# SciML/NonlinearSolve.jl

Hardware: NVIDIA H100
Metric: gmres_jvps_per_s (higher is better)
Workload: dtype f64

## Files before the change

nonlinearsolve.jl_b200/csrc/common.cuh:

```cuda
#pragma once
#include <cuda_runtime.h>
#include <stdint.h>
#include <stdio.h>
#include <string>
#include <vector>
#include "../../include/b200newton.h"

struct b200_ctx {
  int device = 0;
  cudaStream_t stream = nullptr;
  bool own_stream = false;
  int sm_count = 132;
  size_t smem_optin = 0;
  size_t l2_bytes = 0;
  std::string last_error;
  int64_t launches = 0;
  double* d_partials = nullptr;
  double* d_scalars = nullptr;
  double* h_scalars = nullptr;
  void* l2_flush = nullptr;
  size_t l2_flush_bytes = 0;
  cudaStream_t aux_stream = nullptr;
  cudaEvent_t ev_a = nullptr, ev_b = nullptr;
  unsigned long long* d_lu_xchg = nullptr;
  bool prof_on = false;
  struct ProfSlot { double ms = 0, bytes = 0; int64_t launches = 0; } prof[B200_KID_COUNT];
  struct ProfPending { int kid; double bytes; cudaEvent_t a, b; };
  std::vector<ProfPending> prof_pending;
  std::vector<cudaEvent_t> prof_free;
  void prof_begin(int kid, double bytes);
  void prof_end();
  void prof_collect();
  int32_t fail(int32_t code, const char* what, const char* file, int line);
};

#define PLAUNCH(ctx, kid, bytes, kernel, grid, block, smem, ...)                        \
  do {                                                                                  \
    if ((ctx)->prof_on) (ctx)->prof_begin((kid), (bytes));                              \
    kernel<<<(grid), (block), (smem), (ctx)->stream>>>(__VA_ARGS__);                    \
    (ctx)->launches++;                                                                  \
    if ((ctx)->prof_on) (ctx)->prof_end();                                              \
  } while (0)

#define B200_DEVICE_GUARD(ctxexpr)                                                      \
  do {                                                                                  \
    const b200_ctx* g__ = (ctxexpr);                                                    \
    int d__ = -1;                                                                       \
    if (g__ && (cudaGetDevice(&d__) != cudaSuccess || d__ != g__->device)) cudaSetDevice(g__->device); \
  } while (0)

#define B200_RED_MAX_BLOCKS 2048
enum { RED_DOT = 0, RED_SUMSQ = 1, RED_MAXABS = 2, RED_DIFFSQ = 3, RED_MIN = 4, RED_MAX = 5, RED_NEQ = 6,
       RED_SUMSQ2 = 7 , RED_MAXABS2 = 8 , RED_RELVIOL = 9 ,
       RED_COUNT_LE = 10 , RED_COUNT_DIFF_LE = 11  };

#define CUDA_TRY(ctx, expr)                                                             \
  do {                                                                                  \
    cudaError_t e__ = (expr);                                                           \
    if (e__ != cudaSuccess) {                                                           \
      char buf__[512];                                                                  \
      snprintf(buf__, sizeof(buf__), "%s -> %s", #expr, cudaGetErrorString(e__));       \
      return (ctx)->fail(B200_ERR_CUDA, buf__, __FILE__, __LINE__);                     \
    }                                                                                   \
  } while (0)

#define B200_TRY(expr)                  \
  do {                                  \
    int32_t s__ = (expr);               \
    if (s__ != B200_OK) return s__;     \
  } while (0)

#define B200_REQUIRE(ctx, cond, msg)                                                    \
  do {                                                                                  \
    if (!(cond)) return (ctx)->fail(B200_ERR_INVALID, msg, __FILE__, __LINE__);         \
  } while (0)

#define LAUNCH(ctx, kernel, grid, block, smem, ...)                                     \
  do {                                                                                  \
    kernel<<<(grid), (block), (smem), (ctx)->stream>>>(__VA_ARGS__);                    \
    (ctx)->launches++;                                                                  \
  } while (0)

#define CHECK_LAUNCH(ctx) CUDA_TRY(ctx, cudaPeekAtLastError())

__device__ __forceinline__ double warp_sum(double v) {
#pragma unroll
  for (int o = 16; o > 0; o >>= 1) v += __shfl_xor_sync(0xffffffffu, v, o);
  return v;
}
__device__ __forceinline__ double warp_max(double v) {
#pragma unroll
  for (int o = 16; o > 0; o >>= 1) v = fmax(v, __shfl_xor_sync(0xffffffffu, v, o));
  return v;
}
__device__ __forceinline__ double warp_min(double v) {
#pragma unroll
  for (int o = 16; o > 0; o >>= 1) v = fmin(v, __shfl_xor_sync(0xffffffffu, v, o));
  return v;
}
__device__ __forceinline__ double block_sum(double v, double* red) {
  const int lane = threadIdx.x & 31, wid = threadIdx.x >> 5, nw = (blockDim.x + 31) >> 5;
  v = warp_sum(v);
  __syncthreads();
  if (lane == 0) red[wid] = v;
  __syncthreads();
  v = (threadIdx.x < nw) ? red[threadIdx.x] : 0.0;
  if (wid == 0) v = warp_sum(v);
  return v;
}
__device__ __forceinline__ double block_max(double v, double* red) {
  const int lane = threadIdx.x & 31, wid = threadIdx.x >> 5, nw = (blockDim.x + 31) >> 5;
  v = warp_max(v);
  __syncthreads();
  if (lane == 0) red[wid] = v;
  __syncthreads();
  v = (threadIdx.x < nw) ? red[threadIdx.x] : 0.0;
  if (wid == 0) v = warp_max(v);
  return v;
}
__device__ __forceinline__ double abs_nf(double x) {
  double a = fabs(x);
  return (a == a) ? a : __longlong_as_double(0x7ff0000000000000LL);
}
__device__ __forceinline__ void atomic_max_nonneg(double* addr, double v) {
  atomicMax(reinterpret_cast<unsigned long long*>(addr), static_cast<unsigned long long>(__double_as_longlong(v)));
}

struct b200_problem {
  b200_ctx* ctx;
  int32_t kind;
  int32_t N;
  int64_t n;
  double A, B, alpha, a;
  double p;
  const double* pvec;
  b200_residual_cb f_cb;
  b200_jvp_cb jvp_cb, vjp_cb;
  b200_jac_cb jac_dense_cb, jac_nzval_cb;
  void* user;
  double* fd_scratch;
  int64_t *proto_colptr, *proto_rowval;
};

struct b200_sparse_jac;
struct b200_mg;

__device__ __forceinline__ void mbar_init(uint64_t* bar, unsigned count) {
  asm volatile("mbarrier.init.shared::cta.b64 [%0], %1;" ::"r"((unsigned)__cvta_generic_to_shared(bar)), "r"(count));
}
__device__ __forceinline__ void mbar_arrive(uint64_t* bar) {
  asm volatile("mbarrier.arrive.shared::cta.b64 _, [%0];" ::"r"((unsigned)__cvta_generic_to_shared(bar)) : "memory");
}
__device__ __forceinline__ void mbar_expect_tx(uint64_t* bar, unsigned bytes) {
  asm volatile("mbarrier.arrive.expect_tx.shared::cta.b64 _, [%0], %1;" ::"r"((unsigned)__cvta_generic_to_shared(bar)), "r"(bytes) : "memory");
}
__device__ __forceinline__ void mbar_wait(uint64_t* bar, unsigned parity) {
  const unsigned a = (unsigned)__cvta_generic_to_shared(bar);
  unsigned done = 0, spins = 0;
  while (!done) {
    asm volatile("{ .reg .pred p; mbarrier.try_wait.parity.shared::cta.b64 p, [%1], %2; selp.u32 %0, 1, 0, p; }" : "=r"(done) : "r"(a), "r"(parity) : "memory");
    if (++spins > (1u << 26)) break;
  }
}
__device__ __forceinline__ void tma_bulk_load(void* smem_dst, const void* gsrc, unsigned bytes, uint64_t* bar) {
  asm volatile("cp.async.bulk.shared::cluster.global.mbarrier::complete_tx::bytes [%0], [%1], %2, [%3];" ::"r"((unsigned)__cvta_generic_to_shared(smem_dst)),
               "l"(gsrc), "r"(bytes), "r"((unsigned)__cvta_generic_to_shared(bar))
               : "memory");
}
__device__ __forceinline__ void l2_bulk_prefetch(const void* gsrc, unsigned bytes) {
  asm volatile("cp.async.bulk.prefetch.L2.global [%0], %1;" ::"l"(gsrc), "r"(bytes) : "memory");
}

__device__ __forceinline__ void ll_store(unsigned long long* dst, unsigned long long v, unsigned epoch) {
  const unsigned long long e = (unsigned long long)epoch << 32;
  asm volatile("st.relaxed.gpu.global.v2.u64 [%0], {%1, %2};" ::"l"(dst), "l"((v & 0xffffffffull) | e), "l"((v >> 32) | e) : "memory");
}
__device__ __forceinline__ ulonglong2 ll_load(const unsigned long long* src) {
  ulonglong2 p;
  asm volatile("ld.relaxed.gpu.global.v2.u64 {%0, %1}, [%2];" : "=l"(p.x), "=l"(p.y) : "l"(src) : "memory");
  return p;
}
__device__ __forceinline__ void ll_wait(const unsigned long long* src, ulonglong2& p, unsigned epoch, unsigned bound, int* fault) {
  unsigned spins = 0;
  while ((unsigned)(p.x >> 32) != epoch || (unsigned)(p.y >> 32) != epoch) {
    if (++spins > bound) { *fault = 1; break; }
    p = ll_load(src);
  }
}
__device__ __forceinline__ unsigned long long ll_value(ulonglong2 p) { return (p.x & 0xffffffffull) | (p.y << 32); }


constexpr int32_t B200I_ENS_RC_DEFERRED = -7;

struct b200_linop {
  b200_ctx* ctx;
  int32_t kind;
  int64_t n;
  b200_problem* prob;
  const double* u;
  int32_t jvp_mode;
  const int64_t *colptr, *rowval;
  const double* nzval;
  int32_t index_base;
  const double* A;
  int64_t ld;
  b200_matvec_cb mv;
  void* user;
  b200_sparse_jac* sj;
  double shift;
  b200_mg* mg;
  int32_t owns_mg;
  int64_t *csr_rowptr, *csr_col, *csr_map;
  b200_ilu0* ilu;
};
enum { LINOP_PROBLEM = 0, LINOP_CSC = 1, LINOP_DENSE = 2, LINOP_CALLBACK = 3, LINOP_SPARSE_JAC = 4, LINOP_BLOCK_JACOBI = 5, LINOP_MULTIGRID = 6,
       LINOP_ILU0 = 7 };

static inline int32_t b200i_sync_for_callback(b200_ctx* ctx) {
  if (cudaStreamSynchronize(ctx->stream) != cudaSuccess) return B200_ERR_CUDA;
  if (ctx->aux_stream && cudaStreamSynchronize(ctx->aux_stream) != cudaSuccess) return B200_ERR_CUDA;
  return B200_OK;
}
int32_t b200i_linop_apply(b200_linop* op, const double* x, double* y);
int32_t b200i_mg_create(b200_problem* prob, b200_mg** out);
int32_t b200i_mg_destroy(b200_mg* mg);
int32_t b200i_mg_setup(b200_mg* mg, const double* u);
int32_t b200i_mg_apply(b200_mg* mg, const double* x, double* y);
int32_t b200i_mg_levels(b200_mg* mg, int32_t* nlev, int32_t* sizes, int32_t cap);
int32_t b200i_diag_shift(b200_ctx* ctx, int64_t n, double* A, int64_t ld, double shift);
int32_t b200i_qrcp_solve(b200_ctx* ctx, int64_t n, double* A, int64_t ld, double* b, double* x, double* work, int32_t* jpvt_dev, int32_t* rank_host);
int32_t b200i_gram(b200_ctx* ctx, int64_t n, const double* J, int64_t ld, double* C, int64_t ldc);
int32_t b200i_klement_descent(b200_ctx* ctx, int64_t n, const double* J, const double* fu, double* du);
int32_t b200i_klement_update(b200_ctx* ctx, int64_t n, double* J, const double* fu, double* fu_cache, const double* du);
int32_t b200i_ger(b200_ctx* ctx, int64_t n, double* A, int64_t ld, const double* c, const double* w);
int32_t b200i_scaled_identity(b200_ctx* ctx, int64_t n, double* A, int64_t ld, double d);
int32_t b200i_lm_damp(b200_ctx* ctx, int64_t n, double* C, int64_t ldc, double* dtd, double lambda);
void b200i_sparse_jac_csr(b200_sparse_jac* sj, const int64_t** rowptr, const int64_t** csr_col, const int64_t** csr_map);
int32_t b200i_residual_norm(b200_problem* prob, const double* u, double* du, double* d_norminf );
int32_t b200i_axpy_norm(b200_ctx* ctx, int64_t n, double a, const double* x, double* y, double* d_sumsq );
int32_t b200i_reduce_sum_dev(b200_ctx* ctx, int64_t n, const double* x, const double* y, int mode, double* d_out, double a = 0.0);
int32_t b200i_fetch_scalars(b200_ctx* ctx, int count);
```

nonlinearsolve.jl_b200/csrc/gmres.cu:

```cuda
#include "common.cuh"
#include <math.h>
#include <float.h>
#include <stdlib.h>
#include <algorithm>

namespace {
constexpr int GM_THREADS = 256;
constexpr int JT = 8;
constexpr int GM_KCAP = 16384;

struct GmresState {
  int32_t status;
  int32_t k;
  int32_t iter_base;
  int32_t itmax;
  int32_t kmax_cycle;
  int32_t pad;
  double rnorm0, rnorm, tol, atol, rtol, inv_h, hbis;
};

__device__ __forceinline__ void sym_givens(double a, double b, double& c, double& s, double& rho) {
  if (b == 0.0) {
    c = (a == 0.0) ? 1.0 : (a > 0 ? 1.0 : -1.0);
    s = 0.0;
// ... 368 lines not shown
    partial[(int64_t)threadIdx.x * G + blockIdx.x] = s;
  }
}
__global__ void tall_gemvt_final_kernel(int nc, int G, const double* __restrict__ partial, double* __restrict__ y) {
  const int c = threadIdx.x;
  if (c >= nc) return;
  double s = 0.0;
  for (int g = 0; g < G; ++g) s += partial[(int64_t)c * G + g];
  y[c] = s;
}
struct ResidentParams {
  int dim, N, k, passes, G;
  int opkind;
  const int64_t *rowptr, *csr_col, *csr_map;
  const double* nzval;
  int64_t NC;
  int cpc;
  int qs;
  double a, A;
  const double* u;
  const double* const* V;
  double* vnew;
  unsigned long long* slots;
  unsigned epoch_base;
  int* err;
  double* h;
  double* gsub;
  double *R, *cs, *sn, *z, *hraw;
  GmresState* st;
};

constexpr int LL_MAXG = 160;
constexpr int R3_POLLERS = LL_MAXG;
constexpr int R3_SPARE_POLLER = R3_POLLERS - 1;
constexpr int R3_THREADS = 256;
__device__ __forceinline__ void resident_givens_tail(const ResidentParams& P, double hbis, double inv, double* ws, int cap, int tid) {
  const int k = P.k;
  GmresState* st = P.st;
  double* Rk = P.R + (int64_t)(k - 1) * k / 2;
  double* hr = P.hraw ? P.hraw + (int64_t)(k - 1) * (k + 2) / 2 : nullptr;
  const bool staged = 3 * k <= cap;
  double *col, *cs, *sn;
  if (staged) {
    col = ws; cs = ws + k; sn = ws + 2 * k;
    for (int i = tid; i < k; i += R3_THREADS) {
      const double h = P.h[i];
      col[i] = h; cs[i] = P.cs[i]; sn[i] = P.sn[i];
      if (hr) hr[i] = h;
    }
    __syncthreads();
  } else {
    col = Rk; cs = P.cs; sn = P.sn;
    if (tid == 0) {
      for (int i = 0; i < k; ++i) { const double h = P.h[i]; Rk[i] = h; if (hr) hr[i] = h; }
    }
  }
  if (tid == 0) {
    if (hr) hr[k] = hbis;
    double x = col[0];
    for (int i = 0; i + 1 < k; ++i) {
      const double nx = col[i + 1];
      col[i] = cs[i] * x + sn[i] * nx;
      x = sn[i] * x - cs[i] * nx;
    }
    double c, s_, rho;
    sym_givens(x, hbis, c, s_, rho);
    P.cs[k - 1] = c; P.sn[k - 1] = s_; col[k - 1] = rho;
    const double zeta = s_ * P.z[k - 1];
    P.z[k - 1] = c * P.z[k - 1];
    P.z[k] = zeta;
    const double rnorm = fabs(zeta);
    st->rnorm = rnorm; st->hbis = hbis; st->k = k; st->inv_h = inv;
    st->status = *P.err ? B200_LS_NONFINITE : gm_step_status(rnorm, hbis, k, st);
  }
  if (staged) {
    __syncthreads();
    for (int i = tid; i < k; i += R3_THREADS) Rk[i] = col[i];
  }
}

constexpr int R3_RP = 30;
constexpr int R3_ROWS = 2 * R3_RP;
constexpr int R3_RPR = 16;
constexpr int R3_VR = 2 * R3_RPR;
constexpr size_t R3_ANNEX_BYTES = (size_t)(R3_RP - R3_RPR) * R3_THREADS * 16;
constexpr int R3_REPL = 16;
constexpr size_t R3_BUF_WORDS = (size_t)R3_REPL * LL_MAXG * 4;

constexpr unsigned R3_SPIN_BOUND = 1u << 22;

__device__ __forceinline__ void r3_post(unsigned long long* buf, int b, double a, double c, unsigned epoch) {
  const int lane = threadIdx.x;
  if (lane < R3_REPL) {
    unsigned long long* dst = buf + ((size_t)lane * LL_MAXG + b) * 4;
    ll_store(dst, (unsigned long long)__double_as_longlong(a), epoch);
    ll_store(dst + 2, (unsigned long long)__double_as_longlong(c), epoch);
  }
}
__device__ __forceinline__ void r3_poll(const unsigned long long* buf, int b, int G, unsigned epoch, int* err, double* gA, double* gC) {
  const int tid = threadIdx.x;
  if (tid < R3_POLLERS) {
    double xa = 0.0, xc = 0.0;
    if (tid < G) {
      const unsigned long long* src = buf + ((size_t)(b & (R3_REPL - 1)) * LL_MAXG + tid) * 4;
      unsigned long long a0, a1, c0, c1;
      unsigned spins = 0;
      bool ok;
      do {
        asm volatile("ld.relaxed.gpu.global.v2.u64 {%0, %1}, [%2];" : "=l"(a0), "=l"(a1) : "l"(src) : "memory");
        asm volatile("ld.relaxed.gpu.global.v2.u64 {%0, %1}, [%2];" : "=l"(c0), "=l"(c1) : "l"(src + 2) : "memory");
        ok = ((unsigned)(a0 >> 32) == epoch) && ((unsigned)(a1 >> 32) == epoch) && ((unsigned)(c0 >> 32) == epoch) && ((unsigned)(c1 >> 32) == epoch);
        if (++spins > R3_SPIN_BOUND) { *err = 1; break; }
      } while (!ok);
      xa = __longlong_as_double((long long)((a0 & 0xffffffffull) | (a1 << 32)));
      xc = __longlong_as_double((long long)((c0 & 0xffffffffull) | (c1 << 32)));
    }
    xa = warp_sum(xa);
    xc = warp_sum(xc);
    if ((tid & 31) == 0) { gA[tid >> 5] = xa; gC[tid >> 5] = xc; }
  }
}

struct R3Ctx {
  double *stage0, *stage1;
  double2* annex;
  int nrow, ncell, total, k, b, G;
  int qs;
};

__device__ __forceinline__ void r3_issue_smem(const ResidentParams& P, const R3Ctx& cx, uint64_t* mbar, int t, int stage) {
  if (threadIdx.x == 0 && cx.nrow > 0) {
    const double* src = P.V[t % cx.k];
    double* dst = stage ? cx.stage1 : cx.stage0;
    const int srow = min(cx.nrow, 2 * R3_THREADS * cx.qs);
    const int r0 = min(srow, cx.ncell), r1 = srow - r0;
    const int64_t c0 = (int64_t)cx.b * P.cpc;
    mbar_expect_tx(&mbar[stage], (unsigned)srow * 8u);
    tma_bulk_load(dst, src + c0, (unsigned)r0 * 8u, &mbar[stage]);
    if (r1 > 0) tma_bulk_load(dst + cx.ncell, src + P.NC + c0, (unsigned)r1 * 8u, &mbar[stage]);
    if (srow < cx.ncell) l2_bulk_prefetch(src + c0 + srow, (unsigned)(cx.ncell - srow) * 8u);
    if (srow < cx.nrow) {
      const int a = max(srow, cx.ncell) - cx.ncell;
      l2_bulk_prefetch(src + P.NC + c0 + a, (unsigned)(cx.ncell - a) * 8u);
    }
  }
}
#define R3_SMGET(q, lr, sp, gp, o0, o1)                                                                                         \
  do {                                                                                                                            \
    double2 z_;                                                                                                                   \
    if ((q) < cx.qs) z_ = *reinterpret_cast<const double2*>((sp) + (lr));                                                         \
    else z_ = __ldg(reinterpret_cast<const double2*>((gp) + (lr) + (((lr) >= lims) ? hop : (int64_t)0)));                        \
    o0 = z_.x; o1 = z_.y;                                                                                                         \
  } while (0)
__device__ __forceinline__ void r3_issue_regs(const ResidentParams& P, const R3Ctx& cx, int t, double (&vr)[R3_VR]) {
  const double* src = P.V[t % cx.k] + (int64_t)cx.b * P.cpc + 2 * (int)threadIdx.x;
  const int lim = cx.nrow - 2 * (int)threadIdx.x, lims = cx.ncell - 2 * (int)threadIdx.x;
  const int64_t hop = P.NC - cx.ncell;
#pragma unroll
  for (int q = 0; q < R3_RP; ++q) {
    const int lr = 2 * R3_THREADS * q;
    const double* p = src + ((lr >= lims) ? hop : (int64_t)0) + lr;
    if (q < R3_RPR) {
      if (lr < lim) asm volatile("ld.global.nc.L1::no_allocate.v2.f64 {%0, %1}, [%2];" : "=d"(vr[2 * (q < R3_RPR ? q : 0)]), "=d"(vr[2 * (q < R3_RPR ? q : 0) + 1]) : "l"(p));
    } else if (lr < lim) {
      asm volatile("cp.async.cg.shared.global [%0], [%1], 16;" ::"r"((unsigned)__cvta_generic_to_shared(cx.annex + (q - R3_RPR) * R3_THREADS + threadIdx.x)), "l"(p) : "memory");
    }
  }
  asm volatile("cp.async.commit_group;" ::: "memory");
}
#define R3_VRGET(q, o0, o1)                                                                            \
  do {                                                                                                 \
    if ((q) < R3_RPR) { o0 = vr[2 * ((q) < R3_RPR ? (q) : 0)]; o1 = vr[2 * ((q) < R3_RPR ? (q) : 0) + 1]; } \
    else { const double2 z_ = cx.annex[((q) - R3_RPR) * R3_THREADS + threadIdx.x]; o0 = z_.x; o1 = z_.y; }     \
  } while (0)

__device__ __forceinline__ void r3_apply_operator(const ResidentParams& P, const R3Ctx& cx, double (&w)[R3_ROWS]) {
  const int tid = threadIdx.x;
  const double* vk = P.V[P.k - 1];
  const int N = P.N;
  const int64_t NC = P.NC;
  const int ncell = cx.ncell, nrow = cx.nrow;
  const int64_t c0 = (int64_t)cx.b * P.cpc;
  if (P.opkind == 1) {
#pragma unroll
    for (int qq = 0; qq < R3_ROWS; ++qq) {
      const int lr = 2 * (tid + R3_THREADS * (qq >> 1)) + (qq & 1);
      w[qq] = 0.0;
      if (lr < nrow) {
        const int s = lr >= ncell;
        const int64_t r = (int64_t)s * NC + c0 + (lr - s * ncell);
        double acc = 0.0;
        for (int64_t e = P.rowptr[r], e1 = P.rowptr[r + 1]; e < e1; ++e) acc = fma(P.nzval[P.csr_map[e]], vk[P.csr_col[e]], acc);
        w[qq] = acc;
      }
    }
    return;
  }
  const int N2 = N * N, c0i = (int)c0;
  const double invN = 1.0 / (double)N, invN2 = 1.0 / (double)N2;
  const bool d3 = P.dim == 3;
  const double* __restrict__ uu_ = P.u;
#pragma unroll
  for (int q = 0; q < R3_RP; ++q) {
    const int lr = 2 * (tid + R3_THREADS * q);
    w[2 * q] = 0.0;
    w[2 * q + 1] = 0.0;
    if (lr < nrow) {
      const int s = lr >= ncell;
      const int c = c0i + (lr - s * ncell);
      int i, j, kk = 0;
      if (d3) {
        kk = (int)(((double)c + 0.5) * invN2);
        const int r = c - kk * N2;
        j = (int)(((double)r + 0.5) * invN);
        i = r - j * N;
      } else {
        j = (int)(((double)c + 0.5) * invN);
        i = c - j * N;
      }
      const double* x = vk + (int64_t)s * NC + c;
      const double2 xc = *reinterpret_cast<const double2*>(x);
      const double xl = x[(i == 0) ? (N - 1) : -1];
      const double xr = x[(i + 2 == N) ? (2 - N) : 2];
      const int ojm = (j == 0) ? (N - 1) * N : -N, ojp = (j + 1 == N) ? -(N - 1) * N : N;
      const double2 xjm = *reinterpret_cast<const double2*>(x + ojm), xjp = *reinterpret_cast<const double2*>(x + ojp);
      double lap0 = xl + xc.y + xjp.x + xjm.x - 4.0 * xc.x;
      double lap1 = xc.x + xr + xjp.y + xjm.y - 4.0 * xc.y;
      if (d3) {
        const int okm = (kk == 0) ? (N - 1) * N2 : -N2, okp = (kk + 1 == N) ? -(N - 1) * N2 : N2;
        const double2 xkm = *reinterpret_cast<const double2*>(x + okm), xkp = *reinterpret_cast<const double2*>(x + okp);
        lap0 = lap0 + (xkp.x + xkm.x - 2.0 * xc.x);
        lap1 = lap1 + (xkp.y + xkm.y - 2.0 * xc.y);
      }
      const double2 u2 = *reinterpret_cast<const double2*>(uu_ + c), v2 = *reinterpret_cast<const double2*>(uu_ + NC + c);
      const double2 d2 = *reinterpret_cast<const double2*>(vk + c), e2 = *reinterpret_cast<const double2*>(vk + NC + c);
      const double uv0 = 2.0 * u2.x * v2.x, uu0 = u2.x * u2.x, uv1 = 2.0 * u2.y * v2.y, uu1 = u2.y * u2.y;
      w[2 * q] = s ? (P.a * lap0 + (P.A - uv0) * d2.x - uu0 * e2.x) : (P.a * lap0 + (uv0 - (P.A + 1.0)) * d2.x + uu0 * e2.x);
      w[2 * q + 1] = s ? (P.a * lap1 + (P.A - uv1) * d2.y - uu1 * e2.y) : (P.a * lap1 + (uv1 - (P.A + 1.0)) * d2.y + uu1 * e2.y);
    }
  }
}

__device__ __forceinline__ void r3g_poll_issue(const unsigned long long* buf, int b, int G, unsigned long long& a0, unsigned long long& a1) {
  const int tid = threadIdx.x;
  a0 = 0ull; a1 = 0ull;
  if (tid < G) {
    const unsigned long long* src = buf + ((size_t)(b & (R3_REPL - 1)) * LL_MAXG + tid) * 4;
    asm volatile("ld.relaxed.gpu.global.v2.u64 {%0, %1}, [%2];" : "=l"(a0), "=l"(a1) : "l"(src) : "memory");
  }
}
__device__ __forceinline__ void r3g_poll_finish(const unsigned long long* buf, int b, int G, unsigned epoch, int* err, bool need_c, unsigned long long a0,
                                                unsigned long long a1, double* gA, double* gC) {
  const int tid = threadIdx.x;
  if (tid < R3_POLLERS) {
    double xa = 0.0, xc = 0.0;
    if (tid < G) {
      const unsigned long long* src = buf + ((size_t)(b & (R3_REPL - 1)) * LL_MAXG + tid) * 4;
      unsigned spins = 0;
      while (((unsigned)(a0 >> 32) != epoch) || ((unsigned)(a1 >> 32) != epoch)) {
        asm volatile("ld.relaxed.gpu.global.v2.u64 {%0, %1}, [%2];" : "=l"(a0), "=l"(a1) : "l"(src) : "memory");
        if (++spins > R3_SPIN_BOUND) { *err = 1; break; }
      }
      xa = __longlong_as_double((long long)((a0 & 0xffffffffull) | (a1 << 32)));
      if (need_c) {
        unsigned long long c0, c1;
        spins = 0;
        do {
          asm volatile("ld.relaxed.gpu.global.v2.u64 {%0, %1}, [%2];" : "=l"(c0), "=l"(c1) : "l"(src + 2) : "memory");
          if (++spins > R3_SPIN_BOUND) { *err = 1; break; }
        } while (((unsigned)(c0 >> 32) != epoch) || ((unsigned)(c1 >> 32) != epoch));
        xc = __longlong_as_double((long long)((c0 & 0xffffffffull) | (c1 << 32)));
      }
    }
    xa = warp_sum(xa);
    if ((tid & 31) == 0) gA[tid >> 5] = xa;
    if (need_c) {
      xc = warp_sum(xc);
      if ((tid & 31) == 0) gC[tid >> 5] = xc;
    }
  }
}

struct R3GShared {
  uint64_t mbar[2];
  double redA[2][8], redC[2][8];
  double gA[2][8], gC[2][8];
  double hprev[2];
};
static_assert(R3_THREADS == 8 * 32 && R3_POLLERS == 5 * 32, "sum8 / sum5 add the per-warp partials of the CTA / of the polling warps");
__device__ __forceinline__ double sum8(const double* r) { return ((r[0] + r[1]) + (r[2] + r[3])) + ((r[4] + r[5]) + (r[6] + r[7])); }
__device__ __forceinline__ double sum5(const double* g) { return ((g[0] + g[1]) + (g[2] + g[3])) + g[4]; }

template <int ROLE>
__device__ __forceinline__ void r3g_step(const ResidentParams& P, R3Ctx& cx, R3GShared& sh, int t, double (&w)[R3_ROWS], double (&vr)[R3_VR]) {
  constexpr int NEXT = (ROLE + 1) % 3;
  const int tid = threadIdx.x;
  const int par = t & 1;
  const int lim = cx.nrow - 2 * tid;
  const double* sc = (ROLE == 0 ? cx.stage0 : cx.stage1) + 2 * tid;
  const double* sn = (NEXT == 0 ? cx.stage0 : cx.stage1) + 2 * tid;
  const bool more = t + 1 < cx.total;
  const int i = t % cx.k;
  const int lims = cx.ncell - 2 * tid;
  const int64_t hop = P.NC - cx.ncell;
  const double* vcur = P.V[i] + (int64_t)cx.b * P.cpc + 2 * tid;
  const double* vnext = P.V[(t + 1) % cx.k] + (int64_t)cx.b * P.cpc + 2 * tid;
  const unsigned long long* pollbuf = P.slots + (size_t)(t & 3) * R3_BUF_WORDS;
  unsigned long long ea0, ea1;
  r3g_poll_issue(pollbuf, cx.b, cx.G, ea0, ea1);
  if (more) {
    if (NEXT != 2 && cx.nrow > 0) mbar_wait(&sh.mbar[NEXT], (unsigned)(((t + 1) / 3) & 1));
    if (NEXT == 2) asm volatile("cp.async.wait_group 0;" ::: "memory");
    double da = 0.0, dc = 0.0;
    if (i + 1 == cx.k) {
#pragma unroll
      for (int q = 0; q < R3_RP; ++q) {
        const int lr = 2 * R3_THREADS * q;
        if (lr < lim) {
          double x0, x1, y0, y1;
          if (NEXT == 2) { R3_VRGET(q, x0, x1); }
          else { R3_SMGET(q, lr, sn, vnext, x0, x1); }
          if (ROLE == 2) { R3_VRGET(q, y0, y1); }
          else { R3_SMGET(q, lr, sc, vcur, y0, y1); }
          da = fma(x0, w[2 * q], da); da = fma(x1, w[2 * q + 1], da);
          dc = fma(x0, y0, dc); dc = fma(x1, y1, dc);
        }
      }
      dc = warp_sum(dc);
    } else {
      double db = 0.0;
#pragma unroll
      for (int q = 0; q < R3_RP; ++q) {
        const int lr = 2 * R3_THREADS * q;
        if (lr < lim) {
          double x0, x1;
          if (NEXT == 2) { R3_VRGET(q, x0, x1); }
          else { R3_SMGET(q, lr, sn, vnext, x0, x1); }
          da = fma(x0, w[2 * q], da); db = fma(x1, w[2 * q + 1], db);
        }
      }
      da += db;
    }
    da = warp_sum(da);
    if ((tid & 31) == 0) { sh.redA[par][tid >> 5] = da; sh.redC[par][tid >> 5] = dc; }
  }
  if (tid == R3_SPARE_POLLER) sh.gC[par][R3_POLLERS / 32] = (i > 0) ? __ldg(P.gsub + i) : 0.0;
  r3g_poll_finish(pollbuf, cx.b, cx.G, P.epoch_base + (unsigned)t + 1u, P.err, i == 0 && t > 0, ea0, ea1, sh.gA[par], sh.gC[par]);
  __syncthreads();
  if (more && tid < 32) {
    r3_post(P.slots + (size_t)((t + 1) & 3) * R3_BUF_WORDS, cx.b, sum8(sh.redA[par]), sum8(sh.redC[par]), P.epoch_base + (unsigned)(t + 1) + 1u);
  }
  const double* gc = sh.gC[par];
  const double cross = (i > 0) ? gc[R3_POLLERS / 32] : (t > 0 ? sum5(gc) : 0.0);
  const double h = sum5(sh.gA[par]) - sh.hprev[par ^ 1] * cross;
  if (tid == 0) sh.hprev[par] = h;
  if (more) {
#pragma unroll
    for (int q = 0; q < R3_RP; ++q) {
      const int lr = 2 * R3_THREADS * q;
      if (lr < lim) {
        double y0, y1;
        if (ROLE == 2) { R3_VRGET(q, y0, y1); }
        else { R3_SMGET(q, lr, sc, vcur, y0, y1); }
        w[2 * q] = fma(-h, y0, w[2 * q]);
        w[2 * q + 1] = fma(-h, y1, w[2 * q + 1]);
      }
    }
  } else {
    double nacc = 0.0, xacc = 0.0;
#pragma unroll
    for (int q = 0; q < R3_RP; ++q) {
      const int lr = 2 * R3_THREADS * q;
      if (lr < lim) {
        double y0, y1;
        if (ROLE == 2) { R3_VRGET(q, y0, y1); }
        else { R3_SMGET(q, lr, sc, vcur, y0, y1); }
        const double w0 = fma(-h, y0, w[2 * q]), w1 = fma(-h, y1, w[2 * q + 1]);
        w[2 * q] = w0; w[2 * q + 1] = w1;
        nacc = fma(w0, w0, nacc); nacc = fma(w1, w1, nacc);
        xacc = fma(w0, y0, xacc); xacc = fma(w1, y1, xacc);
      }
    }
    nacc = warp_sum(nacc);
    xacc = warp_sum(xacc);
    if ((tid & 31) == 0) { sh.redA[par ^ 1][tid >> 5] = nacc; sh.redC[par ^ 1][tid >> 5] = xacc; }
  }
  if (cx.b == 0 && tid == 0) P.h[i] = (t < cx.k) ? h : P.h[i] + h;
  if (ROLE != 2) {
    if (t + 3 < cx.total) {
      __syncthreads();
      r3_issue_smem(P, cx, sh.mbar, t + 3, ROLE);
    }
  } else if (t + 3 < cx.total) {
    r3_issue_regs(P, cx, t + 3, vr);
  }
}

__global__ void __launch_bounds__(R3_THREADS, 1) resident3g_arnoldi_kernel(ResidentParams P) {
  if (P.st->status != 0) return;
  extern __shared__ __align__(16) double rsm[];
  __shared__ R3GShared sh;
  R3Ctx cx;
  const int cpc = P.cpc;
  const int sw = min(2 * cpc, 2 * R3_THREADS * P.qs);
  cx.stage0 = rsm;
  cx.stage1 = rsm + sw;
  cx.annex = reinterpret_cast<double2*>(rsm + 2 * sw);
  const int tid = threadIdx.x, b = blockIdx.x, G = P.G;
  cx.b = b; cx.G = G; cx.k = P.k; cx.total = P.passes * P.k; cx.qs = P.qs;
  cx.ncell = (int)max((int64_t)0, min((int64_t)cpc, P.NC - (int64_t)b * cpc));
  cx.nrow = 2 * cx.ncell;
  if (tid == 0) {
    mbar_init(&sh.mbar[0], 1);
    mbar_init(&sh.mbar[1], 1);
    asm volatile("fence.mbarrier_init.release.cluster;" ::: "memory");
  }
  __syncthreads();
  r3_issue_smem(P, cx, sh.mbar, 0, 0);
  if (cx.total > 1) r3_issue_smem(P, cx, sh.mbar, 1, 1);
  double w[R3_ROWS];
  double vr[R3_VR];
  r3_apply_operator(P, cx, w);
  const int total = cx.total;
  const int nrow = cx.nrow;
  const int lim = nrow - 2 * tid;
  if (total > 2) r3_issue_regs(P, cx, 2, vr);
  {
    if (nrow > 0) mbar_wait(&sh.mbar[0], 0u);
    const int lims = cx.ncell - 2 * tid;
    const int64_t hop = P.NC - cx.ncell;
    const double* g0 = P.V[0] + (int64_t)b * cpc + 2 * tid;
    double da = 0.0;
#pragma unroll
    for (int q = 0; q < R3_RP; ++q) {
      const int lr = 2 * R3_THREADS * q;
      if (lr < lim) {
        double x0, x1;
        R3_SMGET(q, lr, cx.stage0 + 2 * tid, g0, x0, x1);
        da = fma(x0, w[2 * q], da); da = fma(x1, w[2 * q + 1], da);
      }
    }
    da = warp_sum(da);
    if ((tid & 31) == 0) sh.redA[1][tid >> 5] = da;
    if (tid == 0) sh.hprev[1] = 0.0;
    __syncthreads();
    if (tid < 32) r3_post(P.slots, b, sum8(sh.redA[1]), 0.0, P.epoch_base + 1u);
  }
  for (int t = 0; t < total; t += 3) {
    r3g_step<0>(P, cx, sh, t, w, vr);
    if (t + 1 < total) r3g_step<1>(P, cx, sh, t + 1, w, vr);
    if (t + 2 < total) r3g_step<2>(P, cx, sh, t + 2, w, vr);
  }
  const int par = total & 1;
  __syncthreads();
  if (tid < 32) r3_post(P.slots + (size_t)(total & 3) * R3_BUF_WORDS, b, sum8(sh.redA[par]), sum8(sh.redC[par]), P.epoch_base + (unsigned)total + 1u);
  r3_poll(P.slots + (size_t)(total & 3) * R3_BUF_WORDS, b, G, P.epoch_base + (unsigned)total + 1u, P.err, sh.gA[par], sh.gC[par]);
  __syncthreads();
  const double hbis = sqrt(sum5(sh.gA[par]));
  const double inv = hbis > 0.0 ? 1.0 / hbis : 0.0;
  const int ncell = cx.ncell;
  const int64_t NC = P.NC, c0 = (int64_t)b * cpc;
#pragma unroll
  for (int q = 0; q < R3_RP; ++q) {
    const int lr = 2 * (tid + R3_THREADS * q);
    if (lr < nrow) {
      const int s = lr >= ncell;
      double2 o;
      o.x = w[2 * q] * inv; o.y = w[2 * q + 1] * inv;
      *reinterpret_cast<double2*>(P.vnew + (int64_t)s * NC + c0 + (lr - s * ncell)) = o;
    }
  }
  if (b == 0) {
    if (tid == 0) P.gsub[P.k] = sum5(sh.gC[par]) * inv;
    resident_givens_tail(P, hbis, inv, rsm, 2 * sw, tid);
  }
}
}

struct b200_gmres {
  b200_ctx* ctx;
  int64_t n;
  b200_gmres_opts opts;
  int G;
  int kcap;
  std::vector<double*> V;
  std::vector<double*> slabs;
  double** d_Vptrs;
  int vptr_cap;
  double *w, *r0, *d_h, *d_hacc, *d_R, *d_cs, *d_sn, *d_z, *d_y, *d_partial, *d_norm_partial, *d_norm_partial2;
  double* d_gsub;
  double* d_hraw;
  int64_t hraw_cap;
  GmresState* d_state;
  GmresState* h_state;
  int* d_err;
  unsigned long long* d_slots;
  unsigned ll_epoch;
  b200_linop *Pl, *Pr;
  double *pt1, *pt2;
};

namespace {
int32_t gm_free_arrays(b200_gmres* gm) {
  cudaFree(gm->d_h); cudaFree(gm->d_hacc); cudaFree(gm->d_R); cudaFree(gm->d_cs); cudaFree(gm->d_sn);
  cudaFree(gm->d_z); cudaFree(gm->d_y); cudaFree(gm->d_partial); cudaFree(gm->d_gsub);
  gm->d_h = gm->d_hacc = gm->d_R = gm->d_cs = gm->d_sn = gm->d_z = gm->d_y = gm->d_partial = gm->d_gsub = nullptr;
  return B200_OK;
}

int32_t gm_reserve(b200_gmres* gm, int need) {
  b200_ctx* ctx = gm->ctx;
  if (need <= gm->kcap) return B200_OK;
  int ncap = std::max(need, gm->kcap > 0 ? gm->kcap * 2 : 64);
  const int64_t rsz = (int64_t)ncap * (ncap + 1) / 2;
  double *nh, *nha, *nR, *ncs, *nsn, *nz, *ny, *npart, *ngs;
  CUDA_TRY(ctx, cudaStreamSynchronize(ctx->stream));
  if (cudaMalloc(&nh, sizeof(double) * (ncap + 2)) != cudaSuccess || cudaMalloc(&nha, sizeof(double) * (ncap + 2)) != cudaSuccess ||
      cudaMalloc(&nR, sizeof(double) * rsz) != cudaSuccess || cudaMalloc(&ncs, sizeof(double) * (ncap + 2)) != cudaSuccess ||
      cudaMalloc(&nsn, sizeof(double) * (ncap + 2)) != cudaSuccess || cudaMalloc(&nz, sizeof(double) * (ncap + 2)) != cudaSuccess ||
      cudaMalloc(&ny, sizeof(double) * (ncap + 2)) != cudaSuccess || cudaMalloc(&ngs, sizeof(double) * (ncap + 2)) != cudaSuccess ||
      cudaMalloc(&npart, sizeof(double) * (int64_t)ncap * gm->G) != cudaSuccess) {
    cudaGetLastError();
    return ctx->fail(B200_ERR_NOMEM, "out of device memory growing the Krylov workspace", __FILE__, __LINE__);
  }
  if (gm->kcap > 0) {
    const int oc = gm->kcap;
    CUDA_TRY(ctx, cudaMemcpy(nR, gm->d_R, sizeof(double) * (int64_t)oc * (oc + 1) / 2, cudaMemcpyDeviceToDevice));
    CUDA_TRY(ctx, cudaMemcpy(ncs, gm->d_cs, sizeof(double) * (oc + 2), cudaMemcpyDeviceToDevice));
    CUDA_TRY(ctx, cudaMemcpy(nsn, gm->d_sn, sizeof(double) * (oc + 2), cudaMemcpyDeviceToDevice));
    CUDA_TRY(ctx, cudaMemcpy(nz, gm->d_z, sizeof(double) * (oc + 2), cudaMemcpyDeviceToDevice));
    CUDA_TRY(ctx, cudaMemcpy(ngs, gm->d_gsub, sizeof(double) * (oc + 2), cudaMemcpyDeviceToDevice));
    gm_free_arrays(gm);
  }
  gm->d_h = nh; gm->d_hacc = nha; gm->d_R = nR; gm->d_cs = ncs; gm->d_sn = nsn; gm->d_z = nz; gm->d_y = ny; gm->d_partial = npart; gm->d_gsub = ngs;
  gm->kcap = ncap;
  return B200_OK;
}

constexpr int VSLAB = 16;
int32_t gm_ensure_vector(b200_gmres* gm, int idx) {
  b200_ctx* ctx = gm->ctx;
  bool table_dirty = false;
  const int64_t npad = (gm->n + 1) & ~(int64_t)1;
  while ((int)gm->V.size() <= idx) {
    double* slab = nullptr;
    int cnt = VSLAB;
    if ((int64_t)cnt * npad * 8 > ((int64_t)1 << 31)) cnt = (int)std::max<int64_t>(1, ((int64_t)1 << 31) / (npad * 8));
    CUDA_TRY(ctx, cudaStreamSynchronize(ctx->stream));
    if (cudaMalloc(&slab, sizeof(double) * npad * cnt) != cudaSuccess) {
      cudaGetLastError();
      cnt = 1;
      if (cudaMalloc(&slab, sizeof(double) * npad) != cudaSuccess) {
        cudaGetLastError();
        return B200_ERR_NOMEM;
      }
    }
    CUDA_TRY(ctx, cudaMemsetAsync(slab, 0, sizeof(double) * npad * cnt, ctx->stream));
    gm->slabs.push_back(slab);
    for (int q = 0; q < cnt; ++q) gm->V.push_back(slab + (int64_t)q * npad);
    table_dirty = true;
  }
  if ((int)gm->V.size() > gm->vptr_cap) {
    int ncap = std::max((int)gm->V.size() * 2, 64);
    double** nt = nullptr;
    CUDA_TRY(ctx, cudaStreamSynchronize(ctx->stream));
    CUDA_TRY(ctx, cudaMalloc(&nt, sizeof(double*) * ncap));
    if (gm->d_Vptrs) cudaFree(gm->d_Vptrs);
    gm->d_Vptrs = nt;
    gm->vptr_cap = ncap;
    table_dirty = true;
  }
  if (table_dirty) {
    CUDA_TRY(ctx, cudaMemcpyAsync(gm->d_Vptrs, gm->V.data(), sizeof(double*) * gm->V.size(), cudaMemcpyHostToDevice, ctx->stream));
    CUDA_TRY(ctx, cudaStreamSynchronize(ctx->stream));
  }
  return B200_OK;
}

int32_t gm_fetch_state(b200_gmres* gm) {
  b200_ctx* ctx = gm->ctx;
  CUDA_TRY(ctx, cudaMemcpyAsync(gm->h_state, gm->d_state, sizeof(GmresState), cudaMemcpyDeviceToHost, ctx->stream));
  CUDA_TRY(ctx, cudaStreamSynchronize(ctx->stream));
  return B200_OK;
}
}

namespace {
__global__ void __launch_bounds__(GM_THREADS) block_jacobi_kernel(int64_t NC, double lapdiag, double A, const double* __restrict__ u, const double* __restrict__ x,
                                                                   double* __restrict__ y) {
  const int64_t c = (int64_t)blockIdx.x * blockDim.x + threadIdx.x;
  if (c >= NC) return;
  const double uc = u[c], vc = u[c + NC];
  const double d00 = lapdiag + (2.0 * uc * vc - (A + 1.0)), d01 = uc * uc, d10 = A - 2.0 * uc * vc, d11 = lapdiag - uc * uc;
  const double det = d00 * d11 - d01 * d10;
  const double x0 = x[c], x1 = x[c + NC];
  y[c] = (d11 * x0 - d01 * x1) / det;
  y[c + NC] = (d00 * x1 - d10 * x0) / det;
}
}

static int32_t linop_apply_unshifted(b200_linop* op, const double* x, double* y);
int32_t b200i_linop_apply(b200_linop* op, const double* x, double* y) {
  B200_TRY(linop_apply_unshifted(op, x, y));
  if (op->shift != 0.0) B200_TRY(b200_axpy(op->ctx, op->n, op->shift, x, y));
// ... 537 lines not shown
```

Before: 308.0.

## Stage Krylov vector tails into shared memory slots with cp.async in resident Arnoldi

When a CTA's row count exceeds the shared-memory staged portion, the rows past the staged part used to be read from global memory with __ldg on every pass. They are now copied with cp.async into freed slots of the stage buffers, and the reads are routed through a new slot-aware accessor. The ROLE 1 step also changes its pipeline: it prefetches into L2 and copies tails instead of issuing the TMA load, and ROLE 2 issues the TMA for stage 1 early. Async-proxy fences and mbarrier timeout error reporting are added. This adds complexity and a risk of shared-memory reuse hazards, and it only takes effect for tailed configurations.

```diff
diff --git a/nonlinearsolve.jl_b200/csrc/common.cuh b/nonlinearsolve.jl_b200/csrc/common.cuh
--- a/nonlinearsolve.jl_b200/csrc/common.cuh
+++ b/nonlinearsolve.jl_b200/csrc/common.cuh
@@ -154,12 +154,15 @@
 __device__ __forceinline__ void mbar_expect_tx(uint64_t* bar, unsigned bytes) {
   asm volatile("mbarrier.arrive.expect_tx.shared::cta.b64 _, [%0], %1;" ::"r"((unsigned)__cvta_generic_to_shared(bar)), "r"(bytes) : "memory");
 }
-__device__ __forceinline__ void mbar_wait(uint64_t* bar, unsigned parity) {
+__device__ __forceinline__ void mbar_wait(uint64_t* bar, unsigned parity, int* err = nullptr) {
   const unsigned a = (unsigned)__cvta_generic_to_shared(bar);
   unsigned done = 0, spins = 0;
   while (!done) {
     asm volatile("{ .reg .pred p; mbarrier.try_wait.parity.shared::cta.b64 p, [%1], %2; selp.u32 %0, 1, 0, p; }" : "=r"(done) : "r"(a), "r"(parity) : "memory");
-    if (++spins > (1u << 26)) break;
+    if (++spins > (1u << 26)) {
+      if (err) *err = 1;
+      break;
+    }
   }
 }
 __device__ __forceinline__ void tma_bulk_load(void* smem_dst, const void* gsrc, unsigned bytes, uint64_t* bar) {
@@ -170,6 +173,10 @@
 __device__ __forceinline__ void l2_bulk_prefetch(const void* gsrc, unsigned bytes) {
   asm volatile("cp.async.bulk.prefetch.L2.global [%0], %1;" ::"l"(gsrc), "r"(bytes) : "memory");
 }
+__device__ __forceinline__ void cp_async16(void* smem_dst, const void* gsrc) {
+  asm volatile("cp.async.cg.shared.global [%0], [%1], 16;" ::"r"((unsigned)__cvta_generic_to_shared(smem_dst)), "l"(gsrc) : "memory");
+}
+__device__ __forceinline__ void fence_proxy_async_smem() { asm volatile("fence.proxy.async.shared::cta;" ::: "memory"); }
 
 __device__ __forceinline__ void ll_store(unsigned long long* dst, unsigned long long v, unsigned epoch) {
   const unsigned long long e = (unsigned long long)epoch << 32;
diff --git a/nonlinearsolve.jl_b200/csrc/gmres.cu b/nonlinearsolve.jl_b200/csrc/gmres.cu
--- a/nonlinearsolve.jl_b200/csrc/gmres.cu
+++ b/nonlinearsolve.jl_b200/csrc/gmres.cu
@@ -544,6 +544,34 @@
     else z_ = __ldg(reinterpret_cast<const double2*>((gp) + (lr) + (((lr) >= lims) ? hop : (int64_t)0)));                        \
     o0 = z_.x; o1 = z_.y;                                                                                                         \
   } while (0)
+#define R3_SLOTGET(q, lr, sp, tp, slot, gp, o0, o1)                                                                             \
+  do {                                                                                                                            \
+    double2 z_;                                                                                                                   \
+    if ((q) < cx.qs) z_ = *reinterpret_cast<const double2*>((sp) + (lr));                                                         \
+    else if (slot) {                                                                                                              \
+      if ((q) == cx.qs) asm volatile("cp.async.wait_group 0;" ::: "memory");                                                     \
+      z_ = *reinterpret_cast<const double2*>((tp) + (lr) - 2 * R3_THREADS * cx.qs);                                               \
+    } else z_ = __ldg(reinterpret_cast<const double2*>((gp) + (lr) + (((lr) >= lims) ? hop : (int64_t)0)));                     \
+    o0 = z_.x; o1 = z_.y;                                                                                                         \
+  } while (0)
+__device__ __forceinline__ void r3_prefetch_l2(const ResidentParams& P, const R3Ctx& cx, int t) {
+  if (threadIdx.x == 0 && cx.nrow > 0) {
+    const double* src = P.V[t % cx.k] + (int64_t)cx.b * P.cpc;
+    l2_bulk_prefetch(src, (unsigned)cx.ncell * 8u);
+    l2_bulk_prefetch(src + P.NC, (unsigned)cx.ncell * 8u);
+  }
+}
+constexpr int R3_TAIL_AT = 9;
+__device__ __forceinline__ bool r3_dot_slot(const R3Ctx& cx, int q) { return cx.qs > q / 2; }
+__device__ __forceinline__ bool r3_update_slot(const R3Ctx& cx, int q) { return cx.qs >= R3_TAIL_AT && cx.qs > q - R3_TAIL_AT; }
+__device__ __forceinline__ void r3_tail_copy(const R3Ctx& cx, const double* gp, double* ts, int nslot, int lim, int lims, int64_t hop) {
+  for (int j = 0; j < nslot; ++j) {
+    const int lr = 2 * R3_THREADS * (cx.qs + j);
+    if (lr >= lim) break;
+    cp_async16(ts + 2 * R3_THREADS * j, gp + lr + ((lr >= lims) ? hop : (int64_t)0));
+  }
+  asm volatile("cp.async.commit_group;" ::: "memory");
+}
 __device__ __forceinline__ void r3_issue_regs(const ResidentParams& P, const R3Ctx& cx, int t, double (&vr)[R3_VR]) {
   const double* src = P.V[t % cx.k] + (int64_t)cx.b * P.cpc + 2 * (int)threadIdx.x;
   const int lim = cx.nrow - 2 * (int)threadIdx.x, lims = cx.ncell - 2 * (int)threadIdx.x;
@@ -683,14 +711,15 @@
 __device__ __forceinline__ double sum8(const double* r) { return ((r[0] + r[1]) + (r[2] + r[3])) + ((r[4] + r[5]) + (r[6] + r[7])); }
 __device__ __forceinline__ double sum5(const double* g) { return ((g[0] + g[1]) + (g[2] + g[3])) + g[4]; }
 
-template <int ROLE>
+template <int ROLE, bool TAIL>
 __device__ __forceinline__ void r3g_step(const ResidentParams& P, R3Ctx& cx, R3GShared& sh, int t, double (&w)[R3_ROWS], double (&vr)[R3_VR]) {
   constexpr int NEXT = (ROLE + 1) % 3;
   const int tid = threadIdx.x;
   const int par = t & 1;
   const int lim = cx.nrow - 2 * tid;
-  const double* sc = (ROLE == 0 ? cx.stage0 : cx.stage1) + 2 * tid;
+  double* const sc = (ROLE == 0 ? cx.stage0 : cx.stage1) + 2 * tid;
   const double* sn = (NEXT == 0 ? cx.stage0 : cx.stage1) + 2 * tid;
+  const bool tail = TAIL && lim > 2 * R3_THREADS * cx.qs;
   const bool more = t + 1 < cx.total;
   const int i = t % cx.k;
   const int lims = cx.ncell - 2 * tid;
@@ -701,7 +730,7 @@
   unsigned long long ea0, ea1;
   r3g_poll_issue(pollbuf, cx.b, cx.G, ea0, ea1);
   if (more) {
-    if (NEXT != 2 && cx.nrow > 0) mbar_wait(&sh.mbar[NEXT], (unsigned)(((t + 1) / 3) & 1));
+    if (NEXT != 2 && cx.nrow > 0) mbar_wait(&sh.mbar[NEXT], (unsigned)(((t + 1) / 3) & 1), P.err);
     if (NEXT == 2) asm volatile("cp.async.wait_group 0;" ::: "memory");
     double da = 0.0, dc = 0.0;
     if (i + 1 == cx.k) {
@@ -711,6 +740,7 @@
         if (lr < lim) {
           double x0, x1, y0, y1;
           if (NEXT == 2) { R3_VRGET(q, x0, x1); }
+          else if (NEXT == 0) { R3_SLOTGET(q, lr, sn, cx.stage1 + 2 * tid, TAIL && r3_dot_slot(cx, q), vnext, x0, x1); }
           else { R3_SMGET(q, lr, sn, vnext, x0, x1); }
           if (ROLE == 2) { R3_VRGET(q, y0, y1); }
           else { R3_SMGET(q, lr, sc, vcur, y0, y1); }
@@ -727,6 +757,7 @@
         if (lr < lim) {
           double x0, x1;
           if (NEXT == 2) { R3_VRGET(q, x0, x1); }
+          else if (NEXT == 0) { R3_SLOTGET(q, lr, sn, cx.stage1 + 2 * tid, TAIL && r3_dot_slot(cx, q), vnext, x0, x1); }
           else { R3_SMGET(q, lr, sn, vnext, x0, x1); }
           da = fma(x0, w[2 * q], da); db = fma(x1, w[2 * q + 1], db);
         }
@@ -738,7 +769,9 @@
   }
   if (tid == R3_SPARE_POLLER) sh.gC[par][R3_POLLERS / 32] = (i > 0) ? __ldg(P.gsub + i) : 0.0;
   r3g_poll_finish(pollbuf, cx.b, cx.G, P.epoch_base + (unsigned)t + 1u, P.err, i == 0 && t > 0, ea0, ea1, sh.gA[par], sh.gC[par]);
+  if (ROLE == 2 && tail) fence_proxy_async_smem();
   __syncthreads();
+  if (ROLE == 2 && TAIL && t + 2 < cx.total) r3_issue_smem(P, cx, sh.mbar, t + 2, 1);
   if (more && tid < 32) {
     r3_post(P.slots + (size_t)((t + 1) & 3) * R3_BUF_WORDS, cx.b, sum8(sh.redA[par]), sum8(sh.redC[par]), P.epoch_base + (unsigned)(t + 1) + 1u);
   }
@@ -753,10 +786,11 @@
       if (lr < lim) {
         double y0, y1;
         if (ROLE == 2) { R3_VRGET(q, y0, y1); }
-        else { R3_SMGET(q, lr, sc, vcur, y0, y1); }
+        else { R3_SLOTGET(q, lr, sc, sc, TAIL && r3_update_slot(cx, q), vcur, y0, y1); }
         w[2 * q] = fma(-h, y0, w[2 * q]);
         w[2 * q + 1] = fma(-h, y1, w[2 * q + 1]);
       }
+      if (ROLE != 2 && q + 1 == R3_TAIL_AT && cx.qs >= R3_TAIL_AT && tail) r3_tail_copy(cx, vcur, sc, R3_TAIL_AT, lim, lims, hop);
     }
   } else {
     double nacc = 0.0, xacc = 0.0;
@@ -766,23 +800,28 @@
       if (lr < lim) {
         double y0, y1;
         if (ROLE == 2) { R3_VRGET(q, y0, y1); }
-        else { R3_SMGET(q, lr, sc, vcur, y0, y1); }
+        else { R3_SLOTGET(q, lr, sc, sc, TAIL && r3_update_slot(cx, q), vcur, y0, y1); }
         const double w0 = fma(-h, y0, w[2 * q]), w1 = fma(-h, y1, w[2 * q + 1]);
         w[2 * q] = w0; w[2 * q + 1] = w1;
         nacc = fma(w0, w0, nacc); nacc = fma(w1, w1, nacc);
         xacc = fma(w0, y0, xacc); xacc = fma(w1, y1, xacc);
       }
+      if (ROLE != 2 && q + 1 == R3_TAIL_AT && cx.qs >= R3_TAIL_AT && tail) r3_tail_copy(cx, vcur, sc, R3_TAIL_AT, lim, lims, hop);
     }
     nacc = warp_sum(nacc);
     xacc = warp_sum(xacc);
     if ((tid & 31) == 0) { sh.redA[par ^ 1][tid >> 5] = nacc; sh.redC[par ^ 1][tid >> 5] = xacc; }
   }
   if (cx.b == 0 && tid == 0) P.h[i] = (t < cx.k) ? h : P.h[i] + h;
-  if (ROLE != 2) {
+  if (ROLE == 0 || (ROLE == 1 && !TAIL)) {
     if (t + 3 < cx.total) {
+      if (tail) fence_proxy_async_smem();
       __syncthreads();
       r3_issue_smem(P, cx, sh.mbar, t + 3, ROLE);
     }
+  } else if (ROLE == 1) {
+    if (t + 3 < cx.total) r3_prefetch_l2(P, cx, t + 3);
+    if (t + 2 < cx.total && tail) r3_tail_copy(cx, P.V[(t + 2) % cx.k] + (int64_t)cx.b * P.cpc + 2 * tid, sc, cx.qs, lim, lims, hop);
   } else if (t + 3 < cx.total) {
     r3_issue_regs(P, cx, t + 3, vr);
   }
@@ -818,7 +857,7 @@
   const int lim = nrow - 2 * tid;
   if (total > 2) r3_issue_regs(P, cx, 2, vr);
   {
-    if (nrow > 0) mbar_wait(&sh.mbar[0], 0u);
+    if (nrow > 0) mbar_wait(&sh.mbar[0], 0u, P.err);
     const int lims = cx.ncell - 2 * tid;
     const int64_t hop = P.NC - cx.ncell;
     const double* g0 = P.V[0] + (int64_t)b * cpc + 2 * tid;
@@ -838,10 +877,17 @@
     __syncthreads();
     if (tid < 32) r3_post(P.slots, b, sum8(sh.redA[1]), 0.0, P.epoch_base + 1u);
   }
+  const bool tailed = nrow > 2 * R3_THREADS * cx.qs;
   for (int t = 0; t < total; t += 3) {
-    r3g_step<0>(P, cx, sh, t, w, vr);
-    if (t + 1 < total) r3g_step<1>(P, cx, sh, t + 1, w, vr);
-    if (t + 2 < total) r3g_step<2>(P, cx, sh, t + 2, w, vr);
+    if (tailed) {
+      r3g_step<0, true>(P, cx, sh, t, w, vr);
+      if (t + 1 < total) r3g_step<1, true>(P, cx, sh, t + 1, w, vr);
+      if (t + 2 < total) r3g_step<2, true>(P, cx, sh, t + 2, w, vr);
+    } else {
+      r3g_step<0, false>(P, cx, sh, t, w, vr);
+      if (t + 1 < total) r3g_step<1, false>(P, cx, sh, t + 1, w, vr);
+      if (t + 2 < total) r3g_step<2, false>(P, cx, sh, t + 2, w, vr);
+    }
   }
   const int par = total & 1;
   __syncthreads();
```

After: 366.0, median of 6. 1.19x the previous value.
